# bonjour-l/esa-pose-estimation

Hardware: AMD Instinct MI355X
Metric: HRNet-W32 256x256 crops/sec (heatmaps + fused argmax/refine keypoints) (higher is better)
Workload: dtype bf16x6 (fp32-grade: every f32 operand split exactly into 3 bf16 terms, 6 bf16 MFMAs per product, f32 accumulate; f32 NHWC activations; f32 VALU stem conv1 / output layer) — heat-maps closer to fp64 than the fp32 CPU reference; 1 GPU; seg_hrnet2 HRNet-W32 256x256, batch 32/GPU, 11 keypoints, fp32 NCHW in -> heatmaps -> keypoints (BASELINE configs[1]); global_batch=32, per_gpu_batch=32, parallelism=dp1, hip_graph=True

## Files before the change

### esa-pose-estimation_amd/csrc/head.hip

```cpp
#include "devstate.h"
#include "gaussfit.h"
#include "kernels.h"
#include "refine.h"
#include "sb.h"

namespace esa {
namespace {

constexpr int FTW = 32;
constexpr int FIW = FTW + 2;
constexpr int FROW = FIW + 1;

struct LerpT {
    int i0, i1;
    float l0, l1;
};
__device__ __forceinline__ LerpT lerp_ac_true(int dst, int in, int out) {
    const float scale = out > 1 ? (float)(in - 1) / (float)(out - 1) : 0.f;
    const float src = scale * (float)dst;
    LerpT r;
    r.i0 = min((int)src, in - 1);
    r.i1 = r.i0 + (r.i0 < in - 1 ? 1 : 0);
    r.l1 = src - (float)r.i0;
    r.l0 = 1.f - r.l1;
    return r;
}

__device__ __forceinline__ LerpT lerp_ac_scaled(int dst, int in, float scale) {
    const float src = scale * (float)dst;
    LerpT r;
    r.i0 = min((int)src, in - 1);
    r.i1 = r.i0 + (r.i0 < in - 1 ? 1 : 0);
    r.l1 = src - (float)r.i0;
    r.l0 = 1.f - r.l1;
    return r;
}

__device__ __forceinline__ float final_scale(int in, int out) { return out > 1 ? (float)(in - 1) / (float)(out - 1) : 0.f; }
__device__ __forceinline__ void final_stage8(const FinalParams& p, int n, int gy, int gx, int c8, float sc_y, float sc_x, float v[8]) {
#pragma unroll
    for (int i = 0; i < 8; ++i) v[i] = 0.f;
    if (gy >= 0 && gy < p.H && gx >= 0 && gx < p.W) {
        const LerpT ly = lerp_ac_scaled(gy, p.h, sc_y), lx = lerp_ac_scaled(gx, p.wd, sc_x);
        const size_t r0 = ((size_t)n * p.h + ly.i0) * p.wd, r1 = ((size_t)n * p.h + ly.i1) * p.wd;
        const size_t ps = (size_t)p.Cp * (p.fmt == FMT_BF ? 2 : 4);
        float v00[8], v01[8], v10[8], v11[8];
        auto ld = [&](size_t pix, float v_[8]) {
            if (p.fmt == FMT_BF) {
                unpack8_bf16(*reinterpret_cast<const uint4*>(p.h3 + pix * ps + c8 * 16), v_);
            } else if (p.fmt == FMT_F32) {
                const float* a = reinterpret_cast<const float*>(p.h3 + pix * ps) + c8 * 8;
                const f32x4 a0 = *reinterpret_cast<const f32x4*>(a), a1 = *reinterpret_cast<const f32x4*>(a + 4);
                v_[0] = a0[0]; v_[1] = a0[1]; v_[2] = a0[2]; v_[3] = a0[3]; v_[4] = a1[0]; v_[5] = a1[1]; v_[6] = a1[2]; v_[7] = a1[3];
            } else {
                const char* a = p.h3 + pix * ps + c8 * 32;
                join8(*reinterpret_cast<const uint4*>(a), *reinterpret_cast<const uint4*>(a + 16), v_);
            }
        };
        ld(r0 + lx.i0, v00);
        ld(r0 + lx.i1, v01);
        ld(r1 + lx.i0, v10);
        ld(r1 + lx.i1, v11);
#pragma unroll
        for (int i = 0; i < 8; ++i)
            v[i] = ly.l0 * (lx.l0 * v00[i] + lx.l1 * v01[i]) + ly.l1 * (lx.l0 * v10[i] + lx.l1 * v11[i]);
    }
}
__device__ __forceinline__ float final_stage_raw(const FinalParams& p, int n, int ci, int gy, int gx) {
    float v = 0.f;
    if (gy >= 0 && gy < p.H && gx >= 0 && gx < p.W)
        v = p.x0[(((size_t)n * p.cin + ci) * p.H + gy) * p.W + gx];
    return v;
}

template <int RPT>
__device__ __forceinline__ void final_tile_max(const FinalParams& p, const float* red, int tiles_x, int tiles_y) {
    constexpr int NP = FTW * 8 * RPT;
    const int lane = threadIdx.x & 63;
    const int ntiles = tiles_x * tiles_y, tile = (int)(blockIdx.x % (unsigned)ntiles), n = (int)(blockIdx.x / (unsigned)ntiles);
    const int oy0 = tile / tiles_x * (8 * RPT), ox0 = tile % tiles_x * FTW;
    for (int k = threadIdx.x >> 6; k < p.K; k += 4) {
        float bv = -INFINITY;
        int bi = 0x7fffffff;
#pragma unroll
        for (int j = 0; j < NP / 64; ++j) {
            const int q = lane + 64 * j, oy = oy0 + q / FTW, ox = ox0 + q % FTW;
            if (oy < p.H && ox < p.W) argmax_take(red[k * NP + q], oy * p.W + ox, bv, bi);
        }
#pragma unroll
        for (int off = 32; off >= 1; off >>= 1) {
            const float ov = __shfl_xor(bv, off);
            const int oi = __shfl_xor(bi, off);
            argmax_take(ov, oi, bv, bi);
        }
        if (lane == 0) p.part[((size_t)n * p.K + k) * (size_t)ntiles + tile] = make_float2(bv, __int_as_float(bi));
    }
}

template <int KT, int RPT, bool KP>
__global__ __launch_bounds__(256) void final_kernel(FinalParams p, int tiles_x, int tiles_y) {
    constexpr int FTH = 8 * RPT, FIH = FTH + 2;
    extern __shared__ __attribute__((aligned(16))) char smem[];
    float* tile = reinterpret_cast<float*>(smem);
    const int CT = p.K + p.cin;
    int b = blockIdx.x;
    const int tx = b % tiles_x; b /= tiles_x;
    const int ty = b % tiles_y;
    const int n = b / tiles_y;
    const int oy0 = ty * FTH, ox0 = tx * FTW;

    constexpr int G = (KT + 7) >> 3;
    const float sc_y = final_scale(p.h, p.H), sc_x = final_scale(p.wd, p.W);
    for (int u = threadIdx.x; u < FIH * FIW * G; u += 256) {
        const int c8 = u % G;
        const int q = u / G;
        const int py = q / FIW, px = q - py * FIW;
        const int gy = oy0 - 1 + py, gx = ox0 - 1 + px;
        float v[8];
        final_stage8(p, n, gy, gx, c8, sc_y, sc_x, v);
#pragma unroll
        for (int i = 0; i < 8; ++i) {
            const int c = c8 * 8 + i;
            if (c < p.K) tile[(c * FIH + py) * FROW + px] = v[i];
        }
    }
    for (int u = threadIdx.x; u < FIH * FIW * p.cin; u += 256) {
        const int px = u % FIW;
        const int r = u / FIW;
        const int py = r % FIH, ci = r / FIH;
        tile[((p.K + ci) * FIH + py) * FROW + px] = final_stage_raw(p, n, ci, oy0 - 1 + py, ox0 - 1 + px);
    }
    __syncthreads();

    const int lx = threadIdx.x & (FTW - 1), lyy = (threadIdx.x / FTW) * RPT;
    if constexpr (RPT == 2) {
        f32x2 acc[KT];
#pragma unroll
        for (int k = 0; k < KT; ++k) acc[k] = f32x2{p.bias[k], p.bias[k]};
        for (int c = 0; c < CT; ++c) {
            const float* tp = tile + (c * FIH + lyy) * FROW + lx;
            const float* wp = p.w + (size_t)c * 9 * KT;
            float r[4][3];
#pragma unroll
            for (int i = 0; i < 4; ++i)
#pragma unroll
                for (int j = 0; j < 3; ++j) r[i][j] = tp[i * FROW + j];
#pragma unroll
            for (int tap = 0; tap < 9; ++tap) {
                const f32x2 v = {r[tap / 3][tap % 3], r[tap / 3 + 1][tap % 3]};
#pragma unroll
                for (int k = 0; k < KT; ++k) {
                    const float w = wp[tap * KT + k];
                    acc[k] = __builtin_elementwise_fma(v, f32x2{w, w}, acc[k]);
                }
            }
        }
        const int ox = ox0 + lx;
        if constexpr (KP) {
            __syncthreads();
#pragma unroll
            for (int k = 0; k < KT; ++k)
                if (k < p.K) {
                    tile[k * (FTW * FTH) + lyy * FTW + lx] = acc[k][0];
                    tile[k * (FTW * FTH) + (lyy + 1) * FTW + lx] = acc[k][1];
                }
            __syncthreads();
            final_tile_max<RPT>(p, tile, tiles_x, tiles_y);
            return;
        }
#pragma unroll
        for (int rr = 0; rr < 2; ++rr) {
            const int oy = oy0 + lyy + rr;
            if (oy < p.H && ox < p.W) {
#pragma unroll
                for (int k = 0; k < KT; ++k)
                    if (k < p.K) p.out[(((size_t)n * p.K + k) * p.H + oy) * p.W + ox] = acc[k][rr];
            }
        }
    } else {
        float acc[KT];
#pragma unroll
        for (int k = 0; k < KT; ++k) acc[k] = p.bias[k];
        for (int c = 0; c < CT; ++c) {
            const float* tp = tile + (c * FIH + lyy) * FROW + lx;
            const float* wp = p.w + (size_t)c * 9 * KT;
#pragma unroll
            for (int tap = 0; tap < 9; ++tap) {
                const float v = tp[(tap / 3) * FROW + (tap % 3)];
#pragma unroll
                for (int k = 0; k < KT; ++k) acc[k] = fmaf(v, wp[tap * KT + k], acc[k]);
            }
        }
        const int oy = oy0 + lyy, ox = ox0 + lx;
        if constexpr (KP) {
            __syncthreads();
#pragma unroll
            for (int k = 0; k < KT; ++k)
                if (k < p.K) tile[k * (FTW * FTH) + lyy * FTW + lx] = acc[k];
            __syncthreads();
            final_tile_max<RPT>(p, tile, tiles_x, tiles_y);
            return;
        }
        if (oy < p.H && ox < p.W) {
#pragma unroll
            for (int k = 0; k < KT; ++k)
                if (k < p.K) p.out[(((size_t)n * p.K + k) * p.H + oy) * p.W + ox] = acc[k];
        }
    }
}
template <int KT, int RPT, bool KP = false>
int launch_final_rt(const FinalParams& p, hipStream_t stream) {
    constexpr int FTH = 8 * RPT, FIH = FTH + 2;
    const int tiles_x = (p.W + FTW - 1) / FTW, tiles_y = (p.H + FTH - 1) / FTH;
    const long long nblk = (long long)p.N * tiles_x * tiles_y;
    if (nblk <= 0 || nblk > 0x7fffffffLL) return (int)hipErrorInvalidValue;
    const size_t lds = (size_t)(p.K + p.cin) * FIH * FROW * sizeof(float);
    auto kern = final_kernel<KT, RPT, KP>;
    if (const int e_ = ensure_dyn_lds(reinterpret_cast<const void*>(kern), 64 * 1024)) return e_;
    if (lds > 64 * 1024) return (int)hipErrorInvalidValue;
    hipLaunchKernelGGL(kern, dim3((unsigned)nblk), dim3(256), lds, stream, p, tiles_x, tiles_y);
    return (int)hipGetLastError();
}
inline int final_rpt(int K, int cin, int KT) { return (size_t)(K + cin) * 18 * FROW * sizeof(float) <= 64 * 1024 && KT <= 16 ? 2 : 1; }
template <int KT, bool KP = false>
int launch_final_t(const FinalParams& p, hipStream_t stream) {
    if (final_rpt(p.K, p.cin, KT) == 2) return launch_final_rt<KT, 2, KP>(p, stream);
    return launch_final_rt<KT, 1, KP>(p, stream);
}

constexpr int FKP_MAXC = 40;
__global__ __launch_bounds__(64) void final_kp_finish_kernel(FinalParams p, int kt, int ntiles, float* kp, int* idx_out) {
    __shared__ float sv[81][FKP_MAXC];
    __shared__ float spt[9];
    const int plane = blockIdx.x, n = plane / p.K, k = plane - n * p.K;
    float bv;
    int bi;
    reduce_tile_maxima(p.part + (size_t)plane * ntiles, ntiles, bv, bi);
    const int b0 = bi == 0x7fffffff ? 0 : bi, px = b0 % p.W, py = b0 / p.W;
    const int npt = 1 < px && px < p.W - 2 && 1 < py && py < p.H - 2 ? 9 : 1;
    const int G = (p.K + 7) >> 3, U = G + p.cin, CT = p.K + p.cin;
    const float sc_y = final_scale(p.h, p.H), sc_x = final_scale(p.wd, p.W);
    for (int u = threadIdx.x; u < npt * 9 * U; u += 64) {
        const int j = u % U, slot = u / U, pt = slot / 9, tap = slot - pt * 9;
        const int gy = py + refine_point_dy(pt) - 1 + tap / 3, gx = px + refine_point_dx(pt) - 1 + tap % 3;
        if (j < G) {
            float v[8];
            final_stage8(p, n, gy, gx, j, sc_y, sc_x, v);
#pragma unroll
            for (int i = 0; i < 8; ++i)
                if (j * 8 + i < p.K) sv[slot][j * 8 + i] = v[i];
        } else {
            sv[slot][p.K + j - G] = final_stage_raw(p, n, j - G, gy, gx);
        }
    }
    __syncthreads();
    if ((int)threadIdx.x < npt) {
        float acc = p.bias[k];
        for (int c = 0; c < CT; ++c) {
            const float* wp = p.w + (size_t)c * 9 * kt;
#pragma unroll
            for (int tap = 0; tap < 9; ++tap) acc = fmaf(sv[threadIdx.x * 9 + tap][c], wp[tap * kt + k], acc);
        }
        spt[threadIdx.x] = acc;
    }
    __syncthreads();
    if (threadIdx.x == 0)
        refine_keypoint([&](int yy, int xx) { return spt[refine_point_of(yy - py, xx - px)]; }, p.H, p.W, bi,
                        kp + (size_t)plane * 3, idx_out ? idx_out + plane : nullptr);
}

constexpr int F2V_T = 22, F2V_V = F2V_T + 10, F2V_S = F2V_V + 2;
constexpr int F2V_LDS = 4 * F2V_V * F2V_V * 4 + 4 * F2V_V * F2V_T * 8;
static_assert(F2V_LDS >= 8 * F2V_S * F2V_S * 4, "staging overlay");

template <int S, int NT>
__device__ __forceinline__ void final2_stage_chunk(const FinalParams& p, int n, int g, int G, int sy0, int sx0, float sc_y,
                                                   float sc_x, float* stg, int tid) {
    if (g < G) {
        for (int q = tid; q < S * S; q += NT) {
            float v[8];
            final_stage8(p, n, sy0 + q / S, sx0 + q % S, g, sc_y, sc_x, v);
#pragma unroll
            for (int i = 0; i < 8; ++i) stg[i * S * S + q] = v[i];
        }
    } else {
        for (int u = tid; u < S * S * p.cin; u += NT) {
            const int q = u % (S * S), ci = u / (S * S);
            stg[ci * S * S + q] = final_stage_raw(p, n, ci, sy0 + q / S, sx0 + q % S);
        }
    }
}

template <int KT>
__global__ __launch_bounds__(256) void final2_valu_kernel(FinalParams p, int tiles_x, int ntiles, float* bmax) {
    constexpr int V = F2V_V, T = F2V_T, S = F2V_S;
    __shared__ __attribute__((aligned(16))) char smem[F2V_LDS];
    float* stg = reinterpret_cast<float*>(smem);
    float* val = reinterpret_cast<float*>(smem);
    double* srow = reinterpret_cast<double*>(smem + 4 * V * V * 4);
    const int tid = threadIdx.x, tile = (int)(blockIdx.x % (unsigned)ntiles), n = (int)(blockIdx.x / (unsigned)ntiles);
    const int oy0 = tile / tiles_x * T, ox0 = tile % tiles_x * T, vy0 = oy0 - 5, vx0 = ox0 - 5;
    const float sc_y = final_scale(p.h, p.H), sc_x = final_scale(p.wd, p.W);
    const int G = (p.K + 7) >> 3;
    f32x2 acc[2][KT];
#pragma unroll
    for (int m = 0; m < 2; ++m)
#pragma unroll
        for (int k = 0; k < KT; ++k) acc[m][k] = f32x2{p.bias[k], p.bias[k]};
    for (int g = 0; g <= G; ++g) {
        const int c0 = g < G ? 8 * g : p.K, nc = g < G ? min(8, p.K - 8 * g) : p.cin;
        __syncthreads();
        final2_stage_chunk<S, 256>(p, n, g, G, vy0 - 1, vx0 - 1, sc_y, sc_x, stg, tid);
        __syncthreads();
        for (int i = 0; i < nc; ++i) {
            const float* sp = stg + i * S * S;
            const float* wp = p.w + (size_t)(c0 + i) * 9 * KT;
#pragma unroll 1
            for (int tap = 0; tap < 9; ++tap) {
#pragma unroll
                for (int m = 0; m < 2; ++m) {
                    const int q0 = tid + 512 * m, q1 = q0 + 256, o = (tap / 3) * S + tap % 3;
                    const f32x2 v = {sp[(q0 / V) * S + q0 % V + o], sp[(q1 / V) * S + q1 % V + o]};
#pragma unroll
                    for (int k = 0; k < KT; ++k) {
                        const float w = wp[tap * KT + k];
                        acc[m][k] = __builtin_elementwise_fma(v, f32x2{w, w}, acc[m][k]);
                    }
                }
            }
        }
    }
    const int wv = tid >> 6, lane = tid & 63;
#pragma unroll
    for (int k0 = 0; k0 < KT; k0 += 4) {
        __syncthreads();
// ... 25 lines not shown
        __syncthreads();
        if (k < p.K) {
            for (int i = lane; i < T * T; i += 64) {
                const int r = i / T, c = i % T;
                const float b = (float)blur_taps([&](int t) { return pr[(r + t) * T + c]; });
                if (oy0 + r < p.H && ox0 + c < p.W) bm = max_nan(bm, b);
            }
#pragma unroll
            for (int off = 32; off >= 1; off >>= 1) {
                const float ov = __shfl_xor(bv, off);
                const int oi = __shfl_xor(bi, off);
                argmax_take(ov, oi, bv, bi);
                bm = max_nan(bm, __shfl_xor(bm, off));
            }
            if (lane == 0) {
                const size_t rec = ((size_t)n * p.K + k) * ntiles + tile;
                p.part[rec] = make_float2(bv, __int_as_float(bi));
                bmax[rec] = bm;
            }
        }
    }
}

template <bool HESS>
__global__ __launch_bounds__(64) void final2_valu_finish_kernel(FinalParams p, int kt, int ntiles, const float* bmax, float* kp,
                                                                int* idx_out, double* hess) {
    constexpr int R = 15, S = R + 2;
    __shared__ float stg[8 * S * S];
    __shared__ float win[R * R];
    const int plane = blockIdx.x, n = plane / p.K, k = plane - n * p.K, lane = threadIdx.x;
    float bv;
    int bi;
    reduce_tile_maxima(p.part + (size_t)plane * ntiles, ntiles, bv, bi);
    float bm = -INFINITY;
    for (int t = lane; t < ntiles; t += 64) bm = max_nan(bm, bmax[(size_t)plane * ntiles + t]);
#pragma unroll
    for (int off = 32; off >= 1; off >>= 1) bm = max_nan(bm, __shfl_xor(bm, off));
    if (bi == 0x7fffffff) bi = 0;
    const int px = bi % p.W, py = bi / p.W, wy0 = py - R / 2, wx0 = px - R / 2;
    const float sc_y = final_scale(p.h, p.H), sc_x = final_scale(p.wd, p.W);
    const int G = (p.K + 7) >> 3;
    float acc[4];
#pragma unroll
    for (int j = 0; j < 4; ++j) acc[j] = p.bias[k];
    for (int g = 0; g <= G; ++g) {
        const int c0 = g < G ? 8 * g : p.K, nc = g < G ? min(8, p.K - 8 * g) : p.cin;
        __syncthreads();
        final2_stage_chunk<S, 64>(p, n, g, G, wy0 - 1, wx0 - 1, sc_y, sc_x, stg, lane);
        __syncthreads();
        for (int i = 0; i < nc; ++i) {
            const float* sp = stg + i * S * S;
            const float* wp = p.w + (size_t)(c0 + i) * 9 * kt;
#pragma unroll
            for (int tap = 0; tap < 9; ++tap)
#pragma unroll
                for (int j = 0; j < 4; ++j) {
                    const int q = min(lane + 64 * j, R * R - 1);
                    acc[j] = fmaf(sp[(q / R + tap / 3) * S + q % R + tap % 3], wp[tap * kt + k], acc[j]);
                }
        }
    }
#pragma unroll
    for (int j = 0; j < 4; ++j) {
        const int q = lane + 64 * j, gy = wy0 + q / R, gx = wx0 + q % R;
        if (q < R * R) win[q] = gy >= 0 && gy < p.H && gx >= 0 && gx < p.W ? acc[j] : 0.f;
    }
    __syncthreads();
    final2_finish<HESS>(
        bv, bi, bm, p.H, p.W,
        [&](int j) {
            const int cy = R / 2 + final2_point_dy(j), cx = R / 2 + final2_point_dx(j);
// ... 2 lines not shown
        [&] { return win[(R / 2) * R + R / 2]; }, kp, idx_out, plane, hess);
}

template <bool COV>
__device__ __forceinline__ void final_gf_finish_body(const FinalParams& p, int kt, int ntiles, float* kp, int* idx_out, double* fit,
                                                     int* status, double* hess, double* cov, double* info, double cov_floor) {
    constexpr int R = 2 * GF_R + 1, S = R + 2;
    __shared__ float stg[8 * S * S];
    __shared__ float win[R * R];
    const int plane = blockIdx.x, n = plane / p.K, k = plane - n * p.K, lane = threadIdx.x;
    float bv;
    int bi;
    reduce_tile_maxima(p.part + (size_t)plane * ntiles, ntiles, bv, bi);
    if (bi == 0x7fffffff) bi = 0;
    const int px = bi % p.W, py = bi / p.W, wy0 = py - GF_R, wx0 = px - GF_R;
    const float sc_y = final_scale(p.h, p.H), sc_x = final_scale(p.wd, p.W);
    const int G = (p.K + 7) >> 3;
    float acc[GF_SLOTS];
#pragma unroll
    for (int j = 0; j < GF_SLOTS; ++j) acc[j] = p.bias[k];
    for (int g = 0; g <= G; ++g) {
        const int c0 = g < G ? 8 * g : p.K, nc = g < G ? min(8, p.K - 8 * g) : p.cin;
        __syncthreads();
        final2_stage_chunk<S, 64>(p, n, g, G, wy0 - 1, wx0 - 1, sc_y, sc_x, stg, lane);
        __syncthreads();
        for (int i = 0; i < nc; ++i) {
            const float* sp = stg + i * S * S;
            const float* wp = p.w + (size_t)(c0 + i) * 9 * kt;
#pragma unroll
            for (int tap = 0; tap < 9; ++tap)
#pragma unroll
                for (int j = 0; j < GF_SLOTS; ++j) {
                    const int q = min(lane + 64 * j, R * R - 1);
                    acc[j] = fmaf(sp[(q / R + tap / 3) * S + q % R + tap % 3], wp[tap * kt + k], acc[j]);
                }
        }
    }
#pragma unroll
    for (int j = 0; j < GF_SLOTS; ++j) {
        const int q = lane + 64 * j;
        if (q < R * R) win[q] = acc[j];
    }
    __syncthreads();
    auto at = [&](int yy, int xx) { return win[(yy - wy0) * R + (xx - wx0)]; };
    if (lane == 0) refine_keypoint(at, p.H, p.W, bi, kp + (size_t)plane * 3, idx_out ? idx_out + plane : nullptr);
    if constexpr (COV) gaussfit_plane<true>(at, (size_t)plane, p.H, p.W, bi, kp, fit, status, hess, cov, info, cov_floor);
    else gaussfit_plane(at, (size_t)plane, p.H, p.W, bi, kp, fit, status, hess);
// ... 264 lines not shown
                    d[base + l * 8 + j] = hi;
                    d[base + 512 + l * 8 + j] = lo;
                }
}

int final_kp_tiles(int K, int cin, int H, int W) {
    const int kt = final_kt(K);
    if (kt < 0 || H <= 0 || W <= 0) return 0;
    return ((W + FTW - 1) / FTW) * ((H + 8 * final_rpt(K, cin, kt) - 1) / (8 * final_rpt(K, cin, kt)));
}

int launch_final_kp(const FinalParams& p, float* kp, int* idx_out, hipStream_t stream) {
    const int ntiles = final_kp_tiles(p.K, p.cin, p.H, p.W), kt = final_kt(p.K);
    const long long planes = (long long)p.N * p.K;
    if (!p.part || !kp || ntiles <= 0 || p.K + p.cin > FKP_MAXC || planes > 0x7fffffffLL || (long long)p.H * p.W > 0x7fffffffLL)
        return (int)hipErrorInvalidValue;
    int rc = (int)hipErrorInvalidValue;
    switch (kt) {
        case 11: rc = launch_final_t<11, true>(p, stream); break;
        case 16: rc = launch_final_t<16, true>(p, stream); break;
        case 32: rc = launch_final_t<32, true>(p, stream); break;
    }
    if (rc) return rc;
    hipLaunchKernelGGL(final_kp_finish_kernel, dim3((unsigned)planes), dim3(64), 0, stream, p, kt, ntiles, kp, idx_out);
    return (int)hipGetLastError();
}

int launch_final_gf(const FinalParams& p, float* kp, int* idx_out, double* fit, int* status, double* hess, hipStream_t stream) {
    return launch_final_gf_cov(p, kp, idx_out, fit, status, hess, nullptr, nullptr, 0.0, stream);
}

int launch_final_gf_cov(const FinalParams& p, float* kp, int* idx_out, double* fit, int* status, double* hess, double* cov,
                        double* info, double cov_floor, hipStream_t stream) {
    const int ntiles = final_kp_tiles(p.K, p.cin, p.H, p.W), kt = final_kt(p.K);
    const long long planes = (long long)p.N * p.K;
    if (!p.part || !kp || !status || ntiles <= 0 || kt < 0 || p.cin < 0 || p.cin > 8 || planes > 0x7fffffffLL ||
        (long long)p.H * p.W > 0x7fffffffLL || !(cov_floor >= 0.0))
        return (int)hipErrorInvalidValue;
    int rc = (int)hipErrorInvalidValue;
    switch (kt) {
        case 11: rc = launch_final_t<11, true>(p, stream); break;
        case 16: rc = launch_final_t<16, true>(p, stream); break;
        case 32: rc = launch_final_t<32, true>(p, stream); break;
    }
    if (rc) return rc;
    if (cov || info)
        hipLaunchKernelGGL(final_gfcov_finish_kernel, dim3((unsigned)planes), dim3(64), 0, stream, p, kt, ntiles, kp, idx_out, fit,
                           status, hess, cov, info, cov_floor);
    else
        hipLaunchKernelGGL(final_gf_finish_kernel, dim3((unsigned)planes), dim3(64), 0, stream, p, kt, ntiles, kp, idx_out, fit,
                           status, hess);
    return (int)hipGetLastError();
}

int final2_valu_tiles(int H, int W) {
    if (H <= 0 || W <= 0) return 0;
    return ((H + F2V_T - 1) / F2V_T) * ((W + F2V_T - 1) / F2V_T);
}

int launch_final2_kp(const FinalParams& p, float* bmax, float* kp, int* idx_out, hipStream_t stream, double* hess) {
    const int ntiles = final2_valu_tiles(p.H, p.W), kt = final_kt(p.K);
    const long long planes = (long long)p.N * p.K, nblk = (long long)p.N * ntiles;
    if (!p.part || !bmax || !kp || ntiles <= 0 || kt < 0 || p.cin < 0 || p.cin > 8 || planes > 0x7fffffffLL ||
        nblk > 0x7fffffffLL || (long long)p.H * p.W > 0x7fffffffLL)
        return (int)hipErrorInvalidValue;
    const int tiles_x = (p.W + F2V_T - 1) / F2V_T;
    switch (kt) {
        case 11: hipLaunchKernelGGL(final2_valu_kernel<11>, dim3((unsigned)nblk), dim3(256), 0, stream, p, tiles_x, ntiles, bmax); break;
        case 16: hipLaunchKernelGGL(final2_valu_kernel<16>, dim3((unsigned)nblk), dim3(256), 0, stream, p, tiles_x, ntiles, bmax); break;
        case 32: hipLaunchKernelGGL(final2_valu_kernel<32>, dim3((unsigned)nblk), dim3(256), 0, stream, p, tiles_x, ntiles, bmax); break;
    }
    hipError_t e = hipGetLastError();
    if (e != hipSuccess) return (int)e;
    if (hess)
        hipLaunchKernelGGL(final2_valu_finish_kernel<true>, dim3((unsigned)planes), dim3(64), 0, stream, p, kt, ntiles, bmax, kp,
                           idx_out, hess);
    else
        hipLaunchKernelGGL(final2_valu_finish_kernel<false>, dim3((unsigned)planes), dim3(64), 0, stream, p, kt, ntiles, bmax, kp,
                           idx_out, hess);
    return (int)hipGetLastError();
}

int launch_final(const FinalParams& p, hipStream_t stream) {
    if (p.wpk && final_mfma_supported(p.K, p.cin)) {
        const int cg = (p.K + p.cin + 7) / 8, m = (p.K + 15) / 16;
        if (p.fmt == FMT_HF) {
            switch (cg * 10 + m) {
                case 21: return launch_final_mfma_t<2, 1, true>(p, stream);
                case 31: return launch_final_mfma_t<3, 1, true>(p, stream);
                case 32: return launch_final_mfma_t<3, 2, true>(p, stream);
                case 42: return launch_final_mfma_t<4, 2, true>(p, stream);
                case 52: return launch_final_mfma_t<5, 2, true>(p, stream);
            }
        }
        switch (cg * 10 + m) {
            case 21: return launch_final_mfma_t<2, 1>(p, stream);
            case 31: return launch_final_mfma_t<3, 1>(p, stream);
            case 32: return launch_final_mfma_t<3, 2>(p, stream);
            case 42: return launch_final_mfma_t<4, 2>(p, stream);
            case 52: return launch_final_mfma_t<5, 2>(p, stream);
        }
    }
// ... 11 lines not shown
```

### esa-pose-estimation_amd/csrc/kernels.h

```cpp
#pragma once
#include <hip/hip_runtime.h>
#include <stdint.h>

namespace esa {

enum { FMT_SB = 0, FMT_BF = 1, FMT_F32 = 2, FMT_HF = 3 };
inline bool fmt_half(int fmt) { return fmt == FMT_BF || fmt == FMT_HF; }

int set_error(const char* fmt, ...);

struct ConvParams {
    const char* x;
    char* y;
    const char* res;
    const uint4* w;
    const float* bias;
    int N, H, W, OH, OW;
    int Cinp, Coutp;
    int relu;
    int out_f32;
    int fmt;
    int nheads;
    int x6_reload;
    char* yh[3];
// ... 76 lines not shown

struct FuseParams {
    const char* x[4];
    int h[4], w[4];
    int nterms;
    char* y;
    int N, H, W, Cp;
    int relu;
    int fmt;
};
int launch_fuse(const FuseParams& p, hipStream_t stream);

struct FinalParams {
    const char* h3;
    const float* x0;
    float* out;
    const float* w;
    const float* bias;
    const uint4* wpk;
    int N, H, W, h, wd;
    int K, cin, Cp;
    int fmt;
    float2* part;
};
int launch_final(const FinalParams& p, hipStream_t stream);
int final_kp_tiles(int K, int cin, int H, int W);
int launch_final_kp(const FinalParams& p, float* kp, int* idx_out, hipStream_t stream);
int launch_final_gf(const FinalParams& p, float* kp, int* idx_out, double* fit, int* status, double* hess, hipStream_t stream);
int launch_final_gf_cov(const FinalParams& p, float* kp, int* idx_out, double* fit, int* status, double* hess, double* cov,
                        double* info, double cov_floor, hipStream_t stream);
int final2_valu_tiles(int H, int W);
int launch_final2_kp(const FinalParams& p, float* bmax, float* kp, int* idx_out, hipStream_t stream, double* hess = nullptr);
int final_part_tiles(int K, int cin, int H, int W);
__device__ __forceinline__ void argmax_take(float v, int i, float& bv, int& bi) {
    const bool vn = v != v, bn = bv != bv;
    if (v > bv || (vn && !bn) || ((v == bv || (vn && bn)) && i < bi)) { bv = v; bi = i; }
}
bool final_mfma_supported(int K, int cin);
size_t final_mfma_bytes(int K, int cin);
void pack_final_mfma(const float* w, int K, int cin, void* dst);

struct HeadParams {
    const char* x0;
    const char* t[3];
    char* y;
    const uint4* w0;
// ... 184 lines not shown
```

### esa-pose-estimation_amd/csrc/plan.hip

```cpp
#include <hip/hip_runtime.h>

#include <algorithm>
#include <cmath>
#include <cstdarg>
#include <cstdio>
#include <cstdlib>
#include <cstring>
#include <map>
#include <string>
#include <vector>

#include "../../include/esahrnet.h"
#include "devstate.h"
#include "kernels.h"

namespace esa {
int final_kt(int K);
extern const int kFrontendMaxRows;
int check_boxes_args(const char* who, int m, int frame_h, int frame_w, int scale, int rule);
int check_crops_args(const char* who, int nframes, int pixel_format, float stdv);
int check_cov_args(const char* who, const void* cov_dev, const void* info_dev, double cov_floor);
int check_corr_args(const char* who, int m, int k, int mode);
}

// ... 95 lines not shown
};

struct JobGroup {
    int n = 0;
    int op[6] = {-1, -1, -1, -1, -1, -1};
};

struct ShapePlan {
    int n = 0, h = 0, w = 0;
    bool keep = false;
    size_t bytes = 0;
    std::vector<int> lh, lw;
    bool head2 = false;
    bool head2_ulo = false;
    std::vector<char> multi_on;
    std::vector<char> job_on;
};

enum StemForm { STEM_SEPARATE, STEM_FUSED, STEM_FUSED_X6 };
enum HeadForm { HEAD_UNFUSED, HEAD_SB, HEAD_BF, HEAD_X6 };

struct PlanOptions {
    bool unfused, head_v1, final_valu, no_multihead, no_jobs, no_bblock, no_cbam_jobs, cbam_unfused, stem_pool_separate,
         head3_direct, head3_cout32, bf_unfused_head, bf_head_valu, x6_unfused_head, x6_unfused_stem, x6_reload_weights, tap_all;
    int nlanes;
    int fmt;
    StemForm stem;
    bool fused_block;
    HeadForm head;
    bool head2;
    bool final_mfma;
};

PlanOptions plan_options(const esahrnet_cfg& g) {
    auto on = [](const char* name) { const char* e = getenv(name); return e && e[0] && strcmp(e, "0") != 0; };
    PlanOptions o;
    o.unfused = on("ESAHRNET_UNFUSED"); o.head_v1 = on("ESAHRNET_HEAD_V1"); o.final_valu = on("ESAHRNET_FINAL_VALU");
    o.no_multihead = on("ESAHRNET_NO_MULTIHEAD"); o.no_jobs = on("ESAHRNET_NO_JOBS"); o.no_bblock = on("ESAHRNET_NO_BBLOCK");
    o.no_cbam_jobs = on("ESAHRNET_NO_CBAM_JOBS"); o.cbam_unfused = on("ESAHRNET_CBAM_UNFUSED");
    o.stem_pool_separate = on("ESAHRNET_STEM_POOL_SEPARATE"); o.head3_direct = on("ESAHRNET_HEAD3_DIRECT");
    o.head3_cout32 = on("ESAHRNET_HEAD3_COUT32"); o.bf_unfused_head = on("ESAHRNET_BF_UNFUSED_HEAD");
    o.bf_head_valu = on("ESAHRNET_BF_HEAD_VALU"); o.x6_unfused_head = on("ESAHRNET_X6_UNFUSED_HEAD");
    o.x6_unfused_stem = on("ESAHRNET_X6_UNFUSED_STEM"); o.tap_all = on("ESAHRNET_TAP_ALL");
    o.x6_reload_weights = on("ESAHRNET_X6_RELOAD_WEIGHTS");
    const char* streams = getenv("ESAHRNET_STREAMS");
    o.nlanes = streams && atoi(streams) > 1 ? 4 : 1;
    o.fmt = g.precision == 1 ? esa::FMT_BF : g.precision == 2 ? esa::FMT_F32 : g.precision == 3 ? esa::FMT_HF : esa::FMT_SB;
    const bool sb = o.fmt == esa::FMT_SB, v0 = g.variant == 0;
    const bool x6_stem = esa::stem_fused_x6_supported(g.cin, pad32(g.stem_width), pad32(g.stem_width)) && g.stem_width == 64;
    o.stem = sb && (!v0 || !o.unfused) ? STEM_FUSED
           : o.fmt == esa::FMT_F32 && x6_stem && !o.x6_unfused_stem ? STEM_FUSED_X6 : STEM_SEPARATE;
    o.fused_block = sb && v0 && !o.unfused && !o.no_bblock;
    int nb4 = 0;
    while (nb4 < ESAHRNET_MAX_BRANCHES && g.blocks[3][nb4] > 0) ++nb4;
    const int c0 = pad32(g.widths[0]);
    o.head = !v0 || nb4 != 4 ? HEAD_UNFUSED
           : sb ? (!o.unfused && (c0 == 32 || c0 == 64) ? HEAD_SB : HEAD_UNFUSED)
           : esa::fmt_half(o.fmt) ? (!o.bf_unfused_head && (pad64(g.widths[0]) == 64 || pad64(g.widths[0]) == 128) ? HEAD_BF : HEAD_UNFUSED)
           : !o.x6_unfused_head && (c0 == 32 || c0 == 64) ? HEAD_X6 : HEAD_UNFUSED;
    o.head2 = !o.head_v1 && (o.head != HEAD_SB || ((pad32(g.widths[1]) == 64 || pad32(g.widths[1]) == 96) &&
                                                   esa::head_t_supported(pad32(g.widths[2])) && esa::head_t_supported(pad32(g.widths[3]))));
    o.final_mfma = v0 && o.fmt != esa::FMT_F32 && !o.final_valu && esa::final_mfma_supported(g.num_keypoints, g.cin);
    return o;
}

}

// ... 2035 lines not shown
            p.nterms = o.nterms;
            for (int i = 0; i < o.nterms; ++i) {
                const Tensor& ti = c.tensors[o.terms[i]];
                if (ti.Cp != to.Cp) return fail("plan bug: fuse channel mismatch");
                p.x[i] = T(o.terms[i]); p.h[i] = lh[ti.level]; p.w[i] = lw[ti.level];
            }
            p.y = T(o.out); p.N = n; p.H = lh[to.level]; p.W = lw[to.level]; p.Cp = to.Cp;
            p.relu = o.relu; p.fmt = c.opt.fmt;
            if (desc) {
                describe(desc, c.hf() ? "fuse_kernel<fp16>" : "fuse_kernel", "fuse -> %s", to.tap.c_str());
                desc->bytes = tbytes(o.out);
                for (int i = 0; i < o.nterms; ++i) desc->bytes += tbytes(o.terms[i]);
            } else rc = esa::launch_fuse(p, stream);
            break;
        }
        case OP_FINAL: {
            const Tensor& ti = c.tensors[o.in];
            esa::FinalParams p{};
            p.h3 = T(o.in); p.x0 = static_cast<const float*>(b.x); p.out = static_cast<float*>(b.heat);
            p.w = c.final_w; p.bias = c.final_b; p.wpk = static_cast<const uint4*>(c.final_wpk);
            p.N = n; p.H = height; p.W = width; p.h = lh[ti.level]; p.wd = lw[ti.level];
            p.K = c.cfg.num_keypoints; p.cin = c.cfg.cin; p.Cp = ti.Cp; p.fmt = c.opt.fmt;
            p.part = static_cast<float2*>(b.part);
            if (desc) {
                const ConvSpec& s = c.specs[c.spec_final];
                describe(desc, c.hf() ? "final_kernel<fp16>" : "final_kernel", "%s", s.name.c_str());
                desc->flops = 2.0 * n * height * width * s.cout * s.cin * 9;
                desc->bytes = tbytes(o.in) + (double)n * height * width * (c.cfg.cin + s.cout) * 4;
            } else if (b.req.decoder != DEC_NONE)
                rc = run_decode(c, b, &p, nullptr, 0, 0, n, height, width, stream);
            else rc = esa::launch_final(p, stream);
            break;
        }
    }
    if (rc) return fail("forward: kernel launch failed: %s", hipGetErrorString((hipError_t)rc));
    return 0;
}

static int run_forward(esahrnet_handle h, const void* x_dev, int n, int height, int width, void* heat_dev, void* part_dev,
                       void* ws_dev, size_t ws_bytes, esahrnet_stream stream_, hipEvent_t* events, const Request* req,
                       void* h0_part = nullptr, void* h0_rec = nullptr) {
    if (!h || !x_dev || !(heat_dev || req) || !ws_dev) return fail("forward: null argument");
    if (!h->committed) return fail("forward: esahrnet_commit has not been called");
    if (plan_shape(*h, n, height, width)) return 1;
    const KpScratch ks = kp_scratch(*h, n, height, width, req ? req->decoder : DEC_NONE);
    const size_t need = h->sp.bytes + ks.total();
// ... 1206 lines not shown
```

Baseline: 8324 crops/s.

## Batch and template the final-layer upsample staging loads in the VALU output kernel

```diff
diff --git a/esa-pose-estimation_amd/csrc/head.hip b/esa-pose-estimation_amd/csrc/head.hip
--- a/esa-pose-estimation_amd/csrc/head.hip
+++ b/esa-pose-estimation_amd/csrc/head.hip
@@ -27,6 +27,7 @@
 }
 
 __device__ __forceinline__ LerpT lerp_ac_scaled(int dst, int in, float scale) {
+#pragma clang fp contract(off)
     const float src = scale * (float)dst;
     LerpT r;
     r.i0 = min((int)src, in - 1);
@@ -37,33 +38,58 @@
 }
 
 __device__ __forceinline__ float final_scale(int in, int out) { return out > 1 ? (float)(in - 1) / (float)(out - 1) : 0.f; }
+template <int FMT> constexpr bool final_fmt_half = FMT == FMT_BF || FMT == FMT_HF;
+template <int FMT, typename IDX>
+__device__ __forceinline__ void final_ld8(const char* h3, IDX pix, IDX ps, int c8, uint4& a, uint4& b) {
+    if constexpr (final_fmt_half<FMT>) {
+        a = *reinterpret_cast<const uint4*>(h3 + (pix * ps + (IDX)(c8 * 16)));
+        b = a;
+    } else {
+        const char* s = h3 + (pix * ps + (IDX)(c8 * 32));
+        a = *reinterpret_cast<const uint4*>(s);
+        b = *reinterpret_cast<const uint4*>(s + 16);
+    }
+}
+template <int FMT>
+__device__ __forceinline__ void final_cvt8(const uint4& a, const uint4& b, float v[8]) {
+    static_assert(FMT == FMT_F32 || FMT == FMT_SB || FMT == FMT_BF, "the VALU output layer reads f32, split-bf16 or bf16");
+    if constexpr (FMT == FMT_BF) unpack8_bf16(a, v);
+    else join8_fmt(a, b, v, FMT == FMT_F32);
+}
+__device__ __forceinline__ void final_blend8(const LerpT& ly, const LerpT& lx, const float v00[8], const float v01[8],
+                                             const float v10[8], const float v11[8], float v[8]) {
+#pragma clang fp contract(off)
+#pragma unroll
+    for (int i = 0; i < 6; i += 2) {
+        const float a0 = __builtin_fmaf(lx.l1, v01[i], lx.l0 * v00[i]), b0 = __builtin_fmaf(lx.l1, v11[i], lx.l0 * v10[i]);
+        v[i] = __builtin_fmaf(ly.l1, b0, ly.l0 * a0);
+        const float a1 = __builtin_fmaf(lx.l0, v00[i + 1], lx.l1 * v01[i + 1]), b1 = __builtin_fmaf(lx.l0, v10[i + 1], lx.l1 * v11[i + 1]);
+        v[i + 1] = __builtin_fmaf(ly.l0, a1, ly.l1 * b1);
+    }
+    const float a6 = lx.l0 * v00[6] + lx.l1 * v01[6], b6 = lx.l0 * v10[6] + lx.l1 * v11[6];
+    v[6] = ly.l0 * a6 + ly.l1 * b6;
+    const float a7 = __builtin_fmaf(lx.l1, v01[7], lx.l0 * v00[7]), b7 = __builtin_fmaf(lx.l0, v10[7], lx.l1 * v11[7]);
+    v[7] = ly.l0 * a7 + ly.l1 * b7;
+}
+template <int FMT>
 __device__ __forceinline__ void final_stage8(const FinalParams& p, int n, int gy, int gx, int c8, float sc_y, float sc_x, float v[8]) {
 #pragma unroll
     for (int i = 0; i < 8; ++i) v[i] = 0.f;
     if (gy >= 0 && gy < p.H && gx >= 0 && gx < p.W) {
         const LerpT ly = lerp_ac_scaled(gy, p.h, sc_y), lx = lerp_ac_scaled(gx, p.wd, sc_x);
         const size_t r0 = ((size_t)n * p.h + ly.i0) * p.wd, r1 = ((size_t)n * p.h + ly.i1) * p.wd;
-        const size_t ps = (size_t)p.Cp * (p.fmt == FMT_BF ? 2 : 4);
+        const size_t ps = (size_t)p.Cp * (final_fmt_half<FMT> ? 2 : 4);
         float v00[8], v01[8], v10[8], v11[8];
         auto ld = [&](size_t pix, float v_[8]) {
-            if (p.fmt == FMT_BF) {
-                unpack8_bf16(*reinterpret_cast<const uint4*>(p.h3 + pix * ps + c8 * 16), v_);
-            } else if (p.fmt == FMT_F32) {
-                const float* a = reinterpret_cast<const float*>(p.h3 + pix * ps) + c8 * 8;
-                const f32x4 a0 = *reinterpret_cast<const f32x4*>(a), a1 = *reinterpret_cast<const f32x4*>(a + 4);
-                v_[0] = a0[0]; v_[1] = a0[1]; v_[2] = a0[2]; v_[3] = a0[3]; v_[4] = a1[0]; v_[5] = a1[1]; v_[6] = a1[2]; v_[7] = a1[3];
-            } else {
-                const char* a = p.h3 + pix * ps + c8 * 32;
-                join8(*reinterpret_cast<const uint4*>(a), *reinterpret_cast<const uint4*>(a + 16), v_);
-            }
+            uint4 a, b;
+            final_ld8<FMT>(p.h3, pix, ps, c8, a, b);
+            final_cvt8<FMT>(a, b, v_);
         };
         ld(r0 + lx.i0, v00);
         ld(r0 + lx.i1, v01);
         ld(r1 + lx.i0, v10);
         ld(r1 + lx.i1, v11);
-#pragma unroll
-        for (int i = 0; i < 8; ++i)
-            v[i] = ly.l0 * (lx.l0 * v00[i] + lx.l1 * v01[i]) + ly.l1 * (lx.l0 * v10[i] + lx.l1 * v11[i]);
+        final_blend8(ly, lx, v00, v01, v10, v11, v);
     }
 }
 __device__ __forceinline__ float final_stage_raw(const FinalParams& p, int n, int ci, int gy, int gx) {
@@ -97,8 +123,158 @@
     }
 }
 
-template <int KT, int RPT, bool KP>
-__global__ __launch_bounds__(256) void final_kernel(FinalParams p, int tiles_x, int tiles_y) {
+template <int FMT, int G, int FIH>
+__device__ __forceinline__ void final_stage_tile_serial(const FinalParams& p, float* tile, int n, int oy0, int ox0, float sc_y,
+                                                        float sc_x) {
+    for (int u = threadIdx.x; u < FIH * FIW * G; u += 256) {
+        const int c8 = u % G;
+        const int q = u / G;
+        const int py = q / FIW, px = q - py * FIW;
+        const int gy = oy0 - 1 + py, gx = ox0 - 1 + px;
+        float v[8];
+        final_stage8<FMT>(p, n, gy, gx, c8, sc_y, sc_x, v);
+#pragma unroll
+        for (int i = 0; i < 8; ++i) {
+            const int c = c8 * 8 + i;
+            if (c < p.K) tile[(c * FIH + py) * FROW + px] = v[i];
+        }
+    }
+    for (int u = threadIdx.x; u < FIH * FIW * p.cin; u += 256) {
+        const int px = u % FIW;
+        const int r = u / FIW;
+        const int py = r % FIH, ci = r / FIH;
+        tile[((p.K + ci) * FIH + py) * FROW + px] = final_stage_raw(p, n, ci, oy0 - 1 + py, ox0 - 1 + px);
+    }
+}
+
+constexpr int FUB = 2, FRB = 4;
+__device__ __forceinline__ float final_keep(float v, bool in) { return __uint_as_float(__float_as_uint(v) & (in ? 0xffffffffu : 0u)); }
+struct FinalRawBatch {
+    float v[FRB];
+};
+template <int FIH>
+__device__ __forceinline__ const float* final_raw_unit(const FinalParams& p, int n, int oy0, int ox0, int u, int nr, int& off,
+                                                       bool& in) {
+    const int uc = min(u, nr - 1);
+    const int px = uc % FIW, r = uc / FIW, py = r % FIH, ci = r / FIH;
+    const int gy = oy0 - 1 + py, gx = ox0 - 1 + px;
+    in = gy >= 0 && gy < p.H && gx >= 0 && gx < p.W;
+    off = ((p.K + ci) * FIH + py) * FROW + px;
+    const int cy = min(max(gy, 0), p.H - 1), cx = min(max(gx, 0), p.W - 1);
+    return p.x0 + (((size_t)n * p.cin + ci) * p.H + cy) * p.W + cx;
+}
+template <int FIH>
+__device__ __forceinline__ FinalRawBatch final_raw_load(const FinalParams& p, int n, int oy0, int ox0, int u0, int nr) {
+    const float* src[FRB];
+#pragma unroll
+    for (int j = 0; j < FRB; ++j) {
+        int off;
+        bool in;
+        src[j] = final_raw_unit<FIH>(p, n, oy0, ox0, u0 + 256 * j, nr, off, in);
+    }
+    FinalRawBatch b;
+#pragma unroll
+    for (int j = 0; j < FRB; ++j) b.v[j] = *src[j];
+    return b;
+}
+template <int FIH>
+__device__ __forceinline__ void final_raw_write(const FinalParams& p, float* tile, int n, int oy0, int ox0, int u0, int nr,
+                                                const FinalRawBatch& b, int dump) {
+#pragma unroll
+    for (int j = 0; j < FRB; ++j) {
+        int off;
+        bool in;
+        final_raw_unit<FIH>(p, n, oy0, ox0, u0 + 256 * j, nr, off, in);
+        tile[u0 + 256 * j < nr ? off : dump] = final_keep(b.v[j], in);
+    }
+}
+template <int G, int FIH>
+struct FinalUnit {
+    int c8, py, px, gy, gx;
+    bool live, in;
+    __device__ __forceinline__ FinalUnit(const FinalParams& p, int u, int oy0, int ox0) {
+        constexpr int NU = FIH * FIW * G;
+        live = u < NU;
+        const int uc = min(u, NU - 1), q = uc / G;
+        c8 = uc % G;
+        py = q / FIW;
+        px = q - py * FIW;
+        gy = oy0 - 1 + py;
+        gx = ox0 - 1 + px;
+        in = gy >= 0 && gy < p.H && gx >= 0 && gx < p.W;
+    }
+    __device__ __forceinline__ LerpT lerp_y(const FinalParams& p, float sc_y) const { return lerp_ac_scaled(min(max(gy, 0), p.H - 1), p.h, sc_y); }
+    __device__ __forceinline__ LerpT lerp_x(const FinalParams& p, float sc_x) const { return lerp_ac_scaled(min(max(gx, 0), p.W - 1), p.wd, sc_x); }
+};
+template <int FMT, int G, int FIH>
+__device__ __forceinline__ void final_stage_tile(const FinalParams& p, float* tile, int n, int oy0, int ox0, float sc_y, float sc_x) {
+    constexpr int NU = FIH * FIW * G, NB = (NU + 256 * FUB - 1) / (256 * FUB);
+    const int nr = FIH * FIW * p.cin;
+    const int dump = (p.K + p.cin) * FIH * FROW;
+    for (int u0 = threadIdx.x; u0 < nr; u0 += 256 * FRB) {
+        const FinalRawBatch b = final_raw_load<FIH>(p, n, oy0, ox0, u0, nr);
+        final_raw_write<FIH>(p, tile, n, oy0, ox0, u0, nr, b, dump);
+    }
+    const unsigned ps = (unsigned)p.Cp * (final_fmt_half<FMT> ? 2 : 4);
+    const char* const img = p.h3 + (size_t)n * p.h * p.wd * ps;
+#pragma unroll 1
+    for (int bt = 0; bt < NB; ++bt) {
+        uint4 ra[FUB][4], rb[FUB][4];
+#pragma unroll
+        for (int j = 0; j < FUB; ++j) {
+            const FinalUnit<G, FIH> t(p, (int)threadIdx.x + 256 * (FUB * bt + j), oy0, ox0);
+            const LerpT ly = t.lerp_y(p, sc_y), lx = t.lerp_x(p, sc_x);
+            const unsigned r0 = (unsigned)(ly.i0 * p.wd), r1 = (unsigned)(ly.i1 * p.wd);
+            final_ld8<FMT>(img, r0 + lx.i0, ps, t.c8, ra[j][0], rb[j][0]);
+            final_ld8<FMT>(img, r0 + lx.i1, ps, t.c8, ra[j][1], rb[j][1]);
+            final_ld8<FMT>(img, r1 + lx.i0, ps, t.c8, ra[j][2], rb[j][2]);
+            final_ld8<FMT>(img, r1 + lx.i1, ps, t.c8, ra[j][3], rb[j][3]);
+        }
+        int tid = threadIdx.x;
+        asm("" : "+v"(tid));
+#pragma unroll
+        for (int j = 0; j < FUB; ++j) {
+            const FinalUnit<G, FIH> t(p, tid + 256 * (FUB * bt + j), oy0, ox0);
+            const LerpT ly = t.lerp_y(p, sc_y), lx = t.lerp_x(p, sc_x);
+            float v00[8], v01[8], v10[8], v11[8], v[8];
+            final_cvt8<FMT>(ra[j][0], rb[j][0], v00);
+            final_cvt8<FMT>(ra[j][1], rb[j][1], v01);
+            final_cvt8<FMT>(ra[j][2], rb[j][2], v10);
+            final_cvt8<FMT>(ra[j][3], rb[j][3], v11);
+            final_blend8(ly, lx, v00, v01, v10, v11, v);
+#pragma unroll
+            for (int i = 0; i < 8; ++i) {
+                const int c = t.c8 * 8 + i;
+                tile[t.live && c < p.K ? (c * FIH + t.py) * FROW + t.px : dump] = final_keep(v[i], t.in);
+            }
+        }
+    }
+}
+
+struct FinalArgs {
+    FinalParams p;
+    int tiles_x, tiles_y;
+};
+struct FinalEpilogue {
+    FinalArgs a;
+    int n, oy0, ox0;
+    template <int FTH>
+    __device__ __forceinline__ void read() {
+#if defined(__HIP_DEVICE_COMPILE__)
+        auto* k = (const __attribute__((address_space(4))) FinalArgs*)__builtin_amdgcn_kernarg_segment_ptr();
+        int b = blockIdx.x;
+        asm("" : "+s"(k), "+s"(b));
+        a = *k;
+        ox0 = b % a.tiles_x * FTW; b /= a.tiles_x;
+        oy0 = b % a.tiles_y * FTH;
+        n = b / a.tiles_y;
+#endif
+    }
+};
+
+template <int KT, int RPT, bool KP, int FMT>
+__global__ __launch_bounds__(256) __attribute__((amdgpu_waves_per_eu(KT <= 16 ? 5 : 1)))
+void final_kernel(FinalParams p, int tiles_x, int tiles_y) {
     constexpr int FTH = 8 * RPT, FIH = FTH + 2;
     extern __shared__ __attribute__((aligned(16))) char smem[];
     float* tile = reinterpret_cast<float*>(smem);
@@ -111,25 +287,8 @@
 
     constexpr int G = (KT + 7) >> 3;
     const float sc_y = final_scale(p.h, p.H), sc_x = final_scale(p.wd, p.W);
-    for (int u = threadIdx.x; u < FIH * FIW * G; u += 256) {
-        const int c8 = u % G;
-        const int q = u / G;
-        const int py = q / FIW, px = q - py * FIW;
-        const int gy = oy0 - 1 + py, gx = ox0 - 1 + px;
-        float v[8];
-        final_stage8(p, n, gy, gx, c8, sc_y, sc_x, v);
-#pragma unroll
-        for (int i = 0; i < 8; ++i) {
-            const int c = c8 * 8 + i;
-            if (c < p.K) tile[(c * FIH + py) * FROW + px] = v[i];
-        }
-    }
-    for (int u = threadIdx.x; u < FIH * FIW * p.cin; u += 256) {
-        const int px = u % FIW;
-        const int r = u / FIW;
-        const int py = r % FIH, ci = r / FIH;
-        tile[((p.K + ci) * FIH + py) * FROW + px] = final_stage_raw(p, n, ci, oy0 - 1 + py, ox0 - 1 + px);
-    }
+    if (p.serial_stage) final_stage_tile_serial<FMT, G, FIH>(p, tile, n, oy0, ox0, sc_y, sc_x);
+    else final_stage_tile<FMT, G, FIH>(p, tile, n, oy0, ox0, sc_y, sc_x);
     __syncthreads();
 
     const int lx = threadIdx.x & (FTW - 1), lyy = (threadIdx.x / FTW) * RPT;
@@ -155,27 +314,31 @@
                 }
             }
         }
-        const int ox = ox0 + lx;
+        FinalEpilogue e;
+        e.read<FTH>();
+        const FinalParams& pe = e.a.p;
+        const int ox = e.ox0 + lx;
+        if constexpr (!KP) {
+#pragma unroll
+            for (int rr = 0; rr < 2; ++rr) {
+                const int oy = e.oy0 + lyy + rr;
+                if (oy < pe.H && ox < pe.W) {
+#pragma unroll
+                    for (int k = 0; k < KT; ++k)
+                        if (k < pe.K) pe.out[(((size_t)e.n * pe.K + k) * pe.H + oy) * pe.W + ox] = acc[k][rr];
+                }
+            }
+        }
         if constexpr (KP) {
             __syncthreads();
 #pragma unroll
             for (int k = 0; k < KT; ++k)
-                if (k < p.K) {
+                if (k < pe.K) {
                     tile[k * (FTW * FTH) + lyy * FTW + lx] = acc[k][0];
                     tile[k * (FTW * FTH) + (lyy + 1) * FTW + lx] = acc[k][1];
                 }
             __syncthreads();
-            final_tile_max<RPT>(p, tile, tiles_x, tiles_y);
-            return;
-        }
-#pragma unroll
-        for (int rr = 0; rr < 2; ++rr) {
-            const int oy = oy0 + lyy + rr;
-            if (oy < p.H && ox < p.W) {
-#pragma unroll
-                for (int k = 0; k < KT; ++k)
-                    if (k < p.K) p.out[(((size_t)n * p.K + k) * p.H + oy) * p.W + ox] = acc[k][rr];
-            }
+            final_tile_max<RPT>(pe, tile, e.a.tiles_x, e.a.tiles_y);
         }
     } else {
         float acc[KT];
@@ -191,37 +354,58 @@
                 for (int k = 0; k < KT; ++k) acc[k] = fmaf(v, wp[tap * KT + k], acc[k]);
             }
         }
-        const int oy = oy0 + lyy, ox = ox0 + lx;
+        FinalEpilogue e;
+        e.read<FTH>();
+        const FinalParams& pe = e.a.p;
+        const int oy = e.oy0 + lyy, ox = e.ox0 + lx;
+        if constexpr (!KP) {
+            if (oy < pe.H && ox < pe.W) {
+#pragma unroll
+                for (int k = 0; k < KT; ++k)
+                    if (k < pe.K) pe.out[(((size_t)e.n * pe.K + k) * pe.H + oy) * pe.W + ox] = acc[k];
+            }
+        }
         if constexpr (KP) {
             __syncthreads();
 #pragma unroll
             for (int k = 0; k < KT; ++k)
-                if (k < p.K) tile[k * (FTW * FTH) + lyy * FTW + lx] = acc[k];
+                if (k < pe.K) tile[k * (FTW * FTH) + lyy * FTW + lx] = acc[k];
             __syncthreads();
-            final_tile_max<RPT>(p, tile, tiles_x, tiles_y);
-            return;
-        }
-        if (oy < p.H && ox < p.W) {
-#pragma unroll
-            for (int k = 0; k < KT; ++k)
-                if (k < p.K) p.out[(((size_t)n * p.K + k) * p.H + oy) * p.W + ox] = acc[k];
-        }
-    }
-}
-template <int KT, int RPT, bool KP = false>
-int launch_final_rt(const FinalParams& p, hipStream_t stream) {
+            final_tile_max<RPT>(pe, tile, e.a.tiles_x, e.a.tiles_y);
+        }
+    }
+}
+#define FINAL_FMT_DISPATCH(fmt, CALL)                                    \
+    switch (fmt) {                                                       \
+        case FMT_F32: { constexpr int FMT = FMT_F32; CALL; break; }      \
+        case FMT_SB: { constexpr int FMT = FMT_SB; CALL; break; }        \
+        case FMT_BF: { constexpr int FMT = FMT_BF; CALL; break; }        \
+        default: return (int)hipErrorInvalidValue;                       \
+    }
+template <int KT, int RPT, bool KP, int FMT>
+int launch_final_rtf(const FinalParams& p, hipStream_t stream) {
     constexpr int FTH = 8 * RPT, FIH = FTH + 2;
     const int tiles_x = (p.W + FTW - 1) / FTW, tiles_y = (p.H + FTH - 1) / FTH;
     const long long nblk = (long long)p.N * tiles_x * tiles_y;
     if (nblk <= 0 || nblk > 0x7fffffffLL) return (int)hipErrorInvalidValue;
-    const size_t lds = (size_t)(p.K + p.cin) * FIH * FROW * sizeof(float);
-    auto kern = final_kernel<KT, RPT, KP>;
-    if (const int e_ = ensure_dyn_lds(reinterpret_cast<const void*>(kern), 64 * 1024)) return e_;
+    const size_t lds = (size_t)(p.K + p.cin) * FIH * FROW * sizeof(float) + 16;
     if (lds > 64 * 1024) return (int)hipErrorInvalidValue;
-    hipLaunchKernelGGL(kern, dim3((unsigned)nblk), dim3(256), lds, stream, p, tiles_x, tiles_y);
-    return (int)hipGetLastError();
-}
-inline int final_rpt(int K, int cin, int KT) { return (size_t)(K + cin) * 18 * FROW * sizeof(float) <= 64 * 1024 && KT <= 16 ? 2 : 1; }
+    FinalParams q = p;
+    if ((unsigned long long)p.h * p.wd * p.Cp * 4 > 0xffffffffull) q.serial_stage = 1;
+    auto launch = [&](auto kern) {
+        if (const int e_ = ensure_dyn_lds(reinterpret_cast<const void*>(kern), 64 * 1024)) return e_;
+        hipLaunchKernelGGL(kern, dim3((unsigned)nblk), dim3(256), lds, stream, q, tiles_x, tiles_y);
+        return (int)hipGetLastError();
+    };
+    return launch(final_kernel<KT, RPT, KP, FMT>);
+}
+template <int KT, int RPT, bool KP = false>
+int launch_final_rt(const FinalParams& p, hipStream_t stream) {
+    int rc = 0;
+    FINAL_FMT_DISPATCH(p.fmt, rc = (launch_final_rtf<KT, RPT, KP, FMT>(p, stream)))
+    return rc;
+}
+inline int final_rpt(int K, int cin, int KT) { return (size_t)(K + cin) * 18 * FROW * sizeof(float) + 16 <= 64 * 1024 && KT <= 16 ? 2 : 1; }
 template <int KT, bool KP = false>
 int launch_final_t(const FinalParams& p, hipStream_t stream) {
     if (final_rpt(p.K, p.cin, KT) == 2) return launch_final_rt<KT, 2, KP>(p, stream);
@@ -229,6 +413,7 @@
 }
 
 constexpr int FKP_MAXC = 40;
+template <int FMT>
 __global__ __launch_bounds__(64) void final_kp_finish_kernel(FinalParams p, int kt, int ntiles, float* kp, int* idx_out) {
     __shared__ float sv[81][FKP_MAXC];
     __shared__ float spt[9];
@@ -245,7 +430,7 @@
         const int gy = py + refine_point_dy(pt) - 1 + tap / 3, gx = px + refine_point_dx(pt) - 1 + tap % 3;
         if (j < G) {
             float v[8];
-            final_stage8(p, n, gy, gx, j, sc_y, sc_x, v);
+            final_stage8<FMT>(p, n, gy, gx, j, sc_y, sc_x, v);
 #pragma unroll
             for (int i = 0; i < 8; ++i)
                 if (j * 8 + i < p.K) sv[slot][j * 8 + i] = v[i];
@@ -273,13 +458,13 @@
 constexpr int F2V_LDS = 4 * F2V_V * F2V_V * 4 + 4 * F2V_V * F2V_T * 8;
 static_assert(F2V_LDS >= 8 * F2V_S * F2V_S * 4, "staging overlay");
 
-template <int S, int NT>
+template <int S, int NT, int FMT>
 __device__ __forceinline__ void final2_stage_chunk(const FinalParams& p, int n, int g, int G, int sy0, int sx0, float sc_y,
                                                    float sc_x, float* stg, int tid) {
     if (g < G) {
         for (int q = tid; q < S * S; q += NT) {
             float v[8];
-            final_stage8(p, n, sy0 + q / S, sx0 + q % S, g, sc_y, sc_x, v);
+            final_stage8<FMT>(p, n, sy0 + q / S, sx0 + q % S, g, sc_y, sc_x, v);
 #pragma unroll
             for (int i = 0; i < 8; ++i) stg[i * S * S + q] = v[i];
         }
@@ -291,7 +476,17 @@
     }
 }
 
-template <int KT>
+template <int S, int NT>
+__device__ __forceinline__ void final2_stage_chunk_rt(const FinalParams& p, int n, int g, int G, int sy0, int sx0, float sc_y,
+                                                      float sc_x, float* stg, int tid) {
+    switch (p.fmt) {
+        case FMT_F32: final2_stage_chunk<S, NT, FMT_F32>(p, n, g, G, sy0, sx0, sc_y, sc_x, stg, tid); break;
+        case FMT_BF: final2_stage_chunk<S, NT, FMT_BF>(p, n, g, G, sy0, sx0, sc_y, sc_x, stg, tid); break;
+        default: final2_stage_chunk<S, NT, FMT_SB>(p, n, g, G, sy0, sx0, sc_y, sc_x, stg, tid); break;
+    }
+}
+
+template <int KT, int FMT>
 __global__ __launch_bounds__(256) void final2_valu_kernel(FinalParams p, int tiles_x, int ntiles, float* bmax) {
     constexpr int V = F2V_V, T = F2V_T, S = F2V_S;
     __shared__ __attribute__((aligned(16))) char smem[F2V_LDS];
@@ -310,7 +505,7 @@
     for (int g = 0; g <= G; ++g) {
         const int c0 = g < G ? 8 * g : p.K, nc = g < G ? min(8, p.K - 8 * g) : p.cin;
         __syncthreads();
-        final2_stage_chunk<S, 256>(p, n, g, G, vy0 - 1, vx0 - 1, sc_y, sc_x, stg, tid);
+        final2_stage_chunk<S, 256, FMT>(p, n, g, G, vy0 - 1, vx0 - 1, sc_y, sc_x, stg, tid);
         __syncthreads();
         for (int i = 0; i < nc; ++i) {
             const float* sp = stg + i * S * S;
@@ -382,7 +577,7 @@
     }
 }
 
-template <bool HESS>
+template <bool HESS, int FMT>
 __global__ __launch_bounds__(64) void final2_valu_finish_kernel(FinalParams p, int kt, int ntiles, const float* bmax, float* kp,
                                                                 int* idx_out, double* hess) {
     constexpr int R = 15, S = R + 2;
@@ -406,7 +601,7 @@
     for (int g = 0; g <= G; ++g) {
         const int c0 = g < G ? 8 * g : p.K, nc = g < G ? min(8, p.K - 8 * g) : p.cin;
         __syncthreads();
-        final2_stage_chunk<S, 64>(p, n, g, G, wy0 - 1, wx0 - 1, sc_y, sc_x, stg, lane);
+        final2_stage_chunk<S, 64, FMT>(p, n, g, G, wy0 - 1, wx0 - 1, sc_y, sc_x, stg, lane);
         __syncthreads();
         for (int i = 0; i < nc; ++i) {
             const float* sp = stg + i * S * S;
@@ -455,7 +650,7 @@
     for (int g = 0; g <= G; ++g) {
         const int c0 = g < G ? 8 * g : p.K, nc = g < G ? min(8, p.K - 8 * g) : p.cin;
         __syncthreads();
-        final2_stage_chunk<S, 64>(p, n, g, G, wy0 - 1, wx0 - 1, sc_y, sc_x, stg, lane);
+        final2_stage_chunk_rt<S, 64>(p, n, g, G, wy0 - 1, wx0 - 1, sc_y, sc_x, stg, lane);
         __syncthreads();
         for (int i = 0; i < nc; ++i) {
             const float* sp = stg + i * S * S;
@@ -766,7 +961,8 @@
         case 32: rc = launch_final_t<32, true>(p, stream); break;
     }
     if (rc) return rc;
-    hipLaunchKernelGGL(final_kp_finish_kernel, dim3((unsigned)planes), dim3(64), 0, stream, p, kt, ntiles, kp, idx_out);
+    FINAL_FMT_DISPATCH(p.fmt, hipLaunchKernelGGL(final_kp_finish_kernel<FMT>, dim3((unsigned)planes), dim3(64), 0, stream, p, kt,
+                                                 ntiles, kp, idx_out))
     return (int)hipGetLastError();
 }
 
@@ -809,19 +1005,22 @@
         nblk > 0x7fffffffLL || (long long)p.H * p.W > 0x7fffffffLL)
         return (int)hipErrorInvalidValue;
     const int tiles_x = (p.W + F2V_T - 1) / F2V_T;
+    auto tiles = [&](auto kern) { hipLaunchKernelGGL(kern, dim3((unsigned)nblk), dim3(256), 0, stream, p, tiles_x, ntiles, bmax); };
+    auto finish = [&](auto kern) {
+        hipLaunchKernelGGL(kern, dim3((unsigned)planes), dim3(64), 0, stream, p, kt, ntiles, bmax, kp, idx_out, hess);
+    };
     switch (kt) {
-        case 11: hipLaunchKernelGGL(final2_valu_kernel<11>, dim3((unsigned)nblk), dim3(256), 0, stream, p, tiles_x, ntiles, bmax); break;
-        case 16: hipLaunchKernelGGL(final2_valu_kernel<16>, dim3((unsigned)nblk), dim3(256), 0, stream, p, tiles_x, ntiles, bmax); break;
-        case 32: hipLaunchKernelGGL(final2_valu_kernel<32>, dim3((unsigned)nblk), dim3(256), 0, stream, p, tiles_x, ntiles, bmax); break;
+        case 11: FINAL_FMT_DISPATCH(p.fmt, tiles(final2_valu_kernel<11, FMT>)) break;
+        case 16: FINAL_FMT_DISPATCH(p.fmt, tiles(final2_valu_kernel<16, FMT>)) break;
+        case 32: FINAL_FMT_DISPATCH(p.fmt, tiles(final2_valu_kernel<32, FMT>)) break;
     }
     hipError_t e = hipGetLastError();
     if (e != hipSuccess) return (int)e;
-    if (hess)
-        hipLaunchKernelGGL(final2_valu_finish_kernel<true>, dim3((unsigned)planes), dim3(64), 0, stream, p, kt, ntiles, bmax, kp,
-                           idx_out, hess);
-    else
-        hipLaunchKernelGGL(final2_valu_finish_kernel<false>, dim3((unsigned)planes), dim3(64), 0, stream, p, kt, ntiles, bmax, kp,
-                           idx_out, hess);
+    if (hess) {
+        FINAL_FMT_DISPATCH(p.fmt, finish(final2_valu_finish_kernel<true, FMT>))
+    } else {
+        FINAL_FMT_DISPATCH(p.fmt, finish(final2_valu_finish_kernel<false, FMT>))
+    }
     return (int)hipGetLastError();
 }
 
diff --git a/esa-pose-estimation_amd/csrc/kernels.h b/esa-pose-estimation_amd/csrc/kernels.h
--- a/esa-pose-estimation_amd/csrc/kernels.h
+++ b/esa-pose-estimation_amd/csrc/kernels.h
@@ -122,6 +122,7 @@
     int K, cin, Cp;
     int fmt;
     float2* part;
+    int serial_stage;
 };
 int launch_final(const FinalParams& p, hipStream_t stream);
 int final_kp_tiles(int K, int cin, int H, int W);
diff --git a/esa-pose-estimation_amd/csrc/plan.hip b/esa-pose-estimation_amd/csrc/plan.hip
--- a/esa-pose-estimation_amd/csrc/plan.hip
+++ b/esa-pose-estimation_amd/csrc/plan.hip
@@ -141,7 +141,8 @@
 
 struct PlanOptions {
     bool unfused, head_v1, final_valu, no_multihead, no_jobs, no_bblock, no_cbam_jobs, cbam_unfused, stem_pool_separate,
-         head3_direct, head3_cout32, bf_unfused_head, bf_head_valu, x6_unfused_head, x6_unfused_stem, x6_reload_weights, tap_all;
+         head3_direct, head3_cout32, bf_unfused_head, bf_head_valu, x6_unfused_head, x6_unfused_stem, x6_reload_weights, tap_all,
+         final_serial_stage;
     int nlanes;
     int fmt;
     StemForm stem;
@@ -162,6 +163,7 @@
     o.bf_head_valu = on("ESAHRNET_BF_HEAD_VALU"); o.x6_unfused_head = on("ESAHRNET_X6_UNFUSED_HEAD");
     o.x6_unfused_stem = on("ESAHRNET_X6_UNFUSED_STEM"); o.tap_all = on("ESAHRNET_TAP_ALL");
     o.x6_reload_weights = on("ESAHRNET_X6_RELOAD_WEIGHTS");
+    o.final_serial_stage = on("ESAHRNET_FINAL_SERIAL_STAGE");
     const char* streams = getenv("ESAHRNET_STREAMS");
     o.nlanes = streams && atoi(streams) > 1 ? 4 : 1;
     o.fmt = g.precision == 1 ? esa::FMT_BF : g.precision == 2 ? esa::FMT_F32 : g.precision == 3 ? esa::FMT_HF : esa::FMT_SB;
@@ -2243,6 +2245,7 @@
             p.N = n; p.H = height; p.W = width; p.h = lh[ti.level]; p.wd = lw[ti.level];
             p.K = c.cfg.num_keypoints; p.cin = c.cfg.cin; p.Cp = ti.Cp; p.fmt = c.opt.fmt;
             p.part = static_cast<float2*>(b.part);
+            p.serial_stage = c.opt.final_serial_stage;
             if (desc) {
                 const ConvSpec& s = c.specs[c.spec_final];
                 describe(desc, c.hf() ? "final_kernel<fp16>" : "final_kernel", "%s", s.name.c_str());
```

Result: no change. 8338 crops/s, median of 6 (+0.2%).
